# yccyenchicheng/p2pvg

Measured on NVIDIA H100. Metric: frames/sec (train step, device-timed) MovingMNIST 64x64 seq30, higher is better.
Workload: dtype bf16

## Files before the change

### include/p2pvg_b200.h

```cpp
#ifndef P2PVG_B200_H
#define P2PVG_B200_H
#include <stddef.h>
#include <stdint.h>

#ifdef __cplusplus
extern "C" {
#endif
struct p2pvg_conv_fusion;

#define P2PVG_OK 0
#define P2PVG_ERR_BAD_ARG -1
#define P2PVG_ERR_UNSUPPORTED -2
#define P2PVG_ERR_CUDA -3
#define P2PVG_ERR_WORKSPACE -4

#define P2PVG_F32 0
#define P2PVG_BF16 1

#define P2PVG_ACT_NONE 0
#define P2PVG_ACT_LRELU 1
#define P2PVG_ACT_TANH 2
#define P2PVG_ACT_RELU 4
#define P2PVG_ACT_SIGMOID 3

// ... 27 lines not shown
  int act;
} p2pvg_conv_fusion_t;

int p2pvg_im2col3(const void* x, void* col, int dtype, int N, int H, int W, int C, int ld, int sgn, void* stream);
int p2pvg_col2im3(const void* col, void* y, int dtype, int N, int H, int W, int C, int ld, const float* bias, void* stream);
int p2pvg_maxpool2_fwd(const void* x, void* y, int dtype, int N, int H, int W, int C, void* stream);
int p2pvg_maxpool2_bwd(const void* x, const void* dy, void* dx, int dtype, int N, int H, int W, int C, void* stream);
int p2pvg_upsample2_fwd(const void* x, void* y, int dtype, int N, int H, int W, int C, void* stream);
int p2pvg_upsample2_bwd(const void* dy, void* dx, int dtype, int N, int H, int W, int C, void* stream);
int p2pvg_gather_add(void* dst, int dtype, const float* src, const int* grp_src, int G, int64_t n, void* stream);

int p2pvg_conv_thin_in(const void* x, int dtype, const float* w, const float* bias, void* y, int N, int H, int W, int Ci, int Co,
                       void* stream);
int p2pvg_convT_thin_out(const void* x, int dtype, const float* w, const float* bias, const float* addend, const int* grp_src,
                         int imgs_per_group, void* y, int y_dtype, int N, int H, int W, int Ci, int Co, void* stream);

int p2pvg_im2col_k4s2p1(const void* x, void* col, int dtype, int N, int H, int W, int C, void* stream);
int p2pvg_col2im_k4s2p1(const void* col, const void* col2, const int* grp_src, int imgs_per_group, void* y, int dtype, int N,
                        int Hi, int Wi, int C, const float* bias, int accumulate, void* stream);
int p2pvg_permute4(const void* src, int src_dtype, void* dst, int dst_dtype, const int* dims ,
                   const int64_t* src_strides , int accumulate, void* stream);
int p2pvg_nchw_to_nhwc_dual(const float* src, float* dst_f32, void* dst_act, int act_dtype, int64_t N, int hw, int C, void* stream);
int p2pvg_add_indexed(void* dst, const void* src, int dtype, const int* dst_idx, int F, int64_t n, void* stream);
int p2pvg_group_sum(const void* in, void* out, int dtype, const int* grp_src, int G, int F, int64_t n, void* stream);
int p2pvg_transpose_batched(const void* src, int src_dtype, void* dst, int dst_dtype, int A, int P, int Q, void* stream);
int p2pvg_blockdiag(const void* src, int src_dtype, void* dst, int dst_dtype, int R, int C, int g, void* stream);

size_t p2pvg_bn_workspace_bytes(int G, int C);
int p2pvg_bn_fwd_stats(const void* x, int dtype, int G, int64_t R, int C, const float* gamma, const float* beta, float eps,
                       void* ws, size_t ws_bytes, float* mean, float* invstd, float* var_unbiased, float* scale, float* shift,
// ... 96 lines not shown
```

### p2pvg_b200/_lib.py

```python
from __future__ import annotations

import ctypes
import os

import torch

_HERE = os.path.dirname(os.path.abspath(__file__))
LIB_PATH = os.path.join(_HERE, "libp2pvg_b200.so")

F32, BF16 = 0, 1
ACT_NONE, ACT_LRELU, ACT_TANH, ACT_SIGMOID, ACT_RELU = 0, 1, 2, 3, 4

_lib = None


class KernelError(RuntimeError):
    pass


def load_library():
    global _lib
    if _lib is None:
        if not os.path.exists(LIB_PATH):
            raise ImportError(
# ... 150 lines not shown
            fusion = ctypes.byref(ConvFusion(fwd_stat_partial=stat_partial.data_ptr() if stat_partial is not None else None,
                                             addend_dtype=_dt(addend) if addend is not None else F32,
                                             eval_scale=eval_scale.data_ptr() if eval_scale is not None else None,
                                             eval_shift=eval_shift.data_ptr() if eval_shift is not None else None, act=int(act)))
        self._ck(self.lib.p2pvg_conv_gemm(_i(kind), _p(a), _p(b), _i64(ldb), _p(c), _i(_dt(c)), _i64(ldc), _i(N), _i(H), _i(W), _i(Ck),
                                          _i(Cn), _i(Cm), _p(bias), _p(addend), _p(grp_src), _i(imgs_per_group), _i(int(accumulate)),
                                          _p(ws), _sz(ws.numel()), fusion, self._stream()))

    def conv_thin_in(self, x, w, bias, y, N, H, W, Ci, Co):
        self._ck(self.lib.p2pvg_conv_thin_in(_p(x), _i(_dt(x)), _p(w), _p(bias), _p(y), _i(N), _i(H), _i(W), _i(Ci), _i(Co), self._stream()))

    def convT_thin_out(self, x, w, bias, y, N, H, W, Ci, Co, addend=None, grp_src=None, imgs_per_group=0):
        self._ck(self.lib.p2pvg_convT_thin_out(_p(x), _i(_dt(x)), _p(w), _p(bias), _p(addend), _p(grp_src), _i(imgs_per_group), _p(y),
                                               _i(_dt(y)), _i(N), _i(H), _i(W), _i(Ci), _i(Co), self._stream()))

    def im2col(self, x, col, N, H, W, C):
        self._ck(self.lib.p2pvg_im2col_k4s2p1(_p(x), _p(col), _i(_dt(x)), _i(N), _i(H), _i(W), _i(C), self._stream()))

    def col2im(self, col, y, N, Hi, Wi, C, bias=None, col2=None, grp_src=None, imgs_per_group=0, accumulate=False):
        self._ck(self.lib.p2pvg_col2im_k4s2p1(_p(col), _p(col2), _p(grp_src), _i(imgs_per_group), _p(y), _i(_dt(col)), _i(N),
                                              _i(Hi), _i(Wi), _i(C), _p(bias), _i(int(accumulate)), self._stream()))

    def im2col3(self, x, col, N, H, W, C, ld, sgn=1):
        self._ck(self.lib.p2pvg_im2col3(_p(x), _p(col), _i(_dt(x)), _i(N), _i(H), _i(W), _i(C), _i(ld), _i(sgn), self._stream()))

    def col2im3(self, col, y, N, H, W, C, ld, bias=None):
        self._ck(self.lib.p2pvg_col2im3(_p(col), _p(y), _i(_dt(col)), _i(N), _i(H), _i(W), _i(C), _i(ld), _p(bias), self._stream()))

    def maxpool2_fwd(self, x, y, N, H, W, C):
        self._ck(self.lib.p2pvg_maxpool2_fwd(_p(x), _p(y), _i(_dt(x)), _i(N), _i(H), _i(W), _i(C), self._stream()))
# ... 164 lines not shown
```

### p2pvg_b200/csrc/api.cu

```cuda
#include <stdarg.h>
#include <string.h>

#include "../../include/p2pvg_b200.h"
#include <cstdlib>

#include "common.cuh"

static thread_local char g_err[512] = "";

void p2pvg_set_error(const char* fmt, ...) {
  va_list ap;
  va_start(ap, fmt);
  vsnprintf(g_err, sizeof(g_err), fmt, ap);
  va_end(ap);
}

int p2pvg_check_launch(const char* what) {
  cudaError_t e = cudaPeekAtLastError();
  if (e != cudaSuccess) {
    p2pvg_set_error("%s: %s", what, cudaGetErrorString(e));
    (void)cudaGetLastError();
    return P2PVG_ERR_CUDA;
  }
  return P2PVG_OK;
// ... 8 lines not shown
int p2pvg_gemm_tc_available();
int p2pvg_layernorm_fwd_impl(const float*, const float*, const float*, float*, float*, float*, long long, int, float, cudaStream_t);
int p2pvg_layernorm_bwd_impl(const float*, const float*, const float*, const float*, const float*, float*, float*, float*, long long, int,
                             void*, size_t, cudaStream_t);
int p2pvg_mse_plain_impl(const float*, const float*, const int*, const float*, int, long long, float*, float*, int, cudaStream_t);
int p2pvg_conv_thin_in_impl(const void*, int, const float*, const float*, void*, int, int, int, int, int, cudaStream_t);
int p2pvg_convT_thin_out_impl(const void*, int, const float*, const float*, const float*, const int*, int, void*, int, int, int, int, int,
                              int, cudaStream_t);
int p2pvg_conv_gemm_impl(int, const void*, const void*, long long, void*, int, long long, int, int, int, int, int, int, const float*,
                         const float*, const int*, int, int, void*, size_t, void*, int, const float*, const float*, int, cudaStream_t);
int p2pvg_bn_fwd_finalize_tiles_impl(const void*, int, int, int, int, long long, int, const float*, const float*, float, float*, float*, float*,
                                     float*, float*, cudaStream_t);
int p2pvg_bn_bwd_finalize_tiles_impl(const void*, int, int, int, int, int, float*, float*, cudaStream_t);
int p2pvg_bn_bwd_apply_impl(const void*, const void*, const void*, int, const float*, const float*, const float*, int, long long, int, int,
                            void*, const float*, const float*, const float*, const float*, cudaStream_t);
int p2pvg_im2col_k4s2p1_impl(const void*, void*, int, int, int, int, int, cudaStream_t);
int p2pvg_im2col3_impl(const void*, void*, int, int, int, int, int, int, int, cudaStream_t);
int p2pvg_col2im3_impl(const void*, void*, int, int, int, int, int, int, const float*, cudaStream_t);
int p2pvg_maxpool2_fwd_impl(const void*, void*, int, int, int, int, int, cudaStream_t);
int p2pvg_maxpool2_bwd_impl(const void*, const void*, void*, int, int, int, int, int, cudaStream_t);
int p2pvg_upsample2_fwd_impl(const void*, void*, int, int, int, int, int, cudaStream_t);
int p2pvg_upsample2_bwd_impl(const void*, void*, int, int, int, int, int, cudaStream_t);
int p2pvg_gather_add_impl(void*, int, const float*, const int*, int, long long, cudaStream_t);
int p2pvg_col2im_k4s2p1_impl(const void*, const void*, const int*, int, void*, int, int, int, int, int, const float*, int, cudaStream_t);
int p2pvg_permute4_impl(const void*, int, void*, int, const int*, const long long*, int, cudaStream_t);
int p2pvg_nchw_to_nhwc_dual_impl(const float*, float*, void*, int, long long, int, int, cudaStream_t);
int p2pvg_add_indexed_impl(void*, const void*, int, const int*, int, long long, cudaStream_t);
int p2pvg_group_sum_impl(const void*, void*, int, const int*, int, int, long long, cudaStream_t);
int p2pvg_blockdiag_impl(const void*, int, void*, int, int, int, int, cudaStream_t);
int p2pvg_transpose_batched_impl(const void*, int, void*, int, int, int, int, cudaStream_t);
// ... 88 lines not shown
  P2PVG_REQUIRE(add_dt == P2PVG_F32 || add_dt == P2PVG_BF16, P2PVG_ERR_BAD_ARG, "conv_gemm: bad addend dtype %d", add_dt);
  return p2pvg_conv_gemm_impl(kind, a, b, ldb, c, c_dtype, ldc, N, H, W, Ck, Cn, Cm, bias, reinterpret_cast<const float*>(addend), grp_src,
                              imgs_per_group, accumulate, workspace, ws_bytes, fwd_stat, add_dt, fusion ? fusion->eval_scale : nullptr,
                              fusion ? fusion->eval_shift : nullptr, fusion ? fusion->act : 0, ST);
}

int p2pvg_conv_thin_in(const void* x, int dtype, const float* w, const float* bias, void* y, int N, int H, int W, int Ci, int Co,
                       void* stream) {
  return p2pvg_conv_thin_in_impl(x, dtype, w, bias, y, N, H, W, Ci, Co, ST);
}
int p2pvg_convT_thin_out(const void* x, int dtype, const float* w, const float* bias, const float* addend, const int* grp_src,
                         int imgs_per_group, void* y, int y_dtype, int N, int H, int W, int Ci, int Co, void* stream) {
  return p2pvg_convT_thin_out_impl(x, dtype, w, bias, addend, grp_src, imgs_per_group, y, y_dtype, N, H, W, Ci, Co, ST);
}

int p2pvg_im2col_k4s2p1(const void* x, void* col, int dtype, int N, int H, int W, int C, void* stream) {
  return p2pvg_im2col_k4s2p1_impl(x, col, dtype, N, H, W, C, ST);
}
int p2pvg_col2im_k4s2p1(const void* col, const void* col2, const int* grp_src, int imgs_per_group, void* y, int dtype, int N,
                        int Hi, int Wi, int C, const float* bias, int accumulate, void* stream) {
  return p2pvg_col2im_k4s2p1_impl(col, col2, grp_src, imgs_per_group, y, dtype, N, Hi, Wi, C, bias, accumulate, ST);
}
int p2pvg_permute4(const void* src, int src_dtype, void* dst, int dst_dtype, const int* dims, const int64_t* src_strides,
                   int accumulate, void* stream) {
  return p2pvg_permute4_impl(src, src_dtype, dst, dst_dtype, dims, (const long long*)src_strides, accumulate, ST);
}
int p2pvg_nchw_to_nhwc_dual(const float* src, float* dst_f32, void* dst_act, int act_dtype, int64_t N, int hw, int C, void* stream) {
  return p2pvg_nchw_to_nhwc_dual_impl(src, dst_f32, dst_act, act_dtype, (long long)N, hw, C, ST);
}
int p2pvg_add_indexed(void* dst, const void* src, int dtype, const int* dst_idx, int F, int64_t n, void* stream) {
// ... 168 lines not shown
```

### p2pvg_b200/csrc/bn.cu

```cuda
#include "common.cuh"

#define BN_MAXCHUNK 64

namespace {

__device__ __forceinline__ float act_grad(float y, int act) {
  if (act == P2PVG_ACT_LRELU) return y > 0.f ? 1.f : 0.2f;
  if (act == P2PVG_ACT_TANH) return 1.f - y * y;
  return 1.f;
}

template <typename T, int MODE>
__global__ void __launch_bounds__(256, 3) bn_reduce_kernel(const T* __restrict__ x, const T* __restrict__ dy, const T* __restrict__ y,
                                                        const float* __restrict__ mean, const float* __restrict__ invstd, int act,
                                                        long long R, int C, int rows_per_chunk, double2* __restrict__ partial,
                                                        const float* __restrict__ scale, const float* __restrict__ shift) {
  constexpr int V = VecN<T>::N;
  const int CV = C / V;
  const int lanes = 256 / CV;
  const int cv = threadIdx.x % CV, lane = threadIdx.x / CV;
  const int g = blockIdx.y, chunk = blockIdx.x, nchunk = gridDim.x;
  const long long r0 = (long long)chunk * rows_per_chunk;
  long long r1 = r0 + rows_per_chunk;
  if (r1 > R) r1 = R;
// ... 358 lines not shown
                "bn_bwd: y may only be omitted for LeakyReLU with scale/shift supplied");
  const int vec = dtype == P2PVG_BF16 ? 8 : 4;
  if (int e = check_bn_shape(C, vec, "bn_bwd")) return e;
  P2PVG_REQUIRE(ws_bytes >= p2pvg_bn_workspace_bytes_impl(G, C), P2PVG_ERR_WORKSPACE, "bn_bwd: workspace too small");
  if (G == 0) return P2PVG_OK;
  Chunking ch = choose_chunks(R, C, vec);
  dim3 grid(ch.nchunk, G);
  DISPATCH_DTYPE(dtype, T, (bn_reduce_kernel<T, 1><<<grid, 256, 0, st>>>((const T*)x, (const T*)dy, (const T*)y, mean, invstd, act, R, C,
                                                                         ch.rows_per_chunk, (double2*)ws, scale, shift)));
  bn_bwd_finalize_kernel<<<cdiv((long long)G * C, 256), 256, 0, st>>>((const double2*)ws, ch.nchunk, G, C, sum_dz, sum_dzx);
  DISPATCH_DTYPE(dtype, T, (bn_bwd_apply_kernel<T><<<grid, 256, 0, st>>>((const T*)dy, (const T*)x, (const T*)y, mean, invstd, gamma, sum_dz,
                                                                         sum_dzx, R, C, ch.rows_per_chunk, act, (T*)dx, scale, shift)));
  return p2pvg_check_launch("bn_bwd");
}

int p2pvg_bn_param_grad_impl(const float* sum_dz, const float* sum_dzx, int G, int C, float* dgamma, float* dbeta, cudaStream_t st) {
  bn_param_grad_kernel<<<cdiv(C, 128), 128, 0, st>>>(sum_dz, sum_dzx, G, C, dgamma, dbeta);
  return p2pvg_check_launch("bn_param_grad");
}

int p2pvg_bn_ema_impl(float* rmean, float* rvar, const float* mean, const float* var_unbiased, const int* order, int ncalls, int C,
                      float momentum, cudaStream_t st) {
  bn_ema_kernel<<<cdiv(C, 128), 128, 0, st>>>(rmean, rvar, mean, var_unbiased, order, ncalls, C, momentum);
  return p2pvg_check_launch("bn_ema");
}

int p2pvg_bn_eval_coeffs_impl(const float* gamma, const float* beta, const float* rmean, const float* rvar, float eps, int C, float* scale,
                              float* shift, cudaStream_t st) {
  bn_eval_coeffs_kernel<<<cdiv(C, 128), 128, 0, st>>>(gamma, beta, rmean, rvar, eps, C, scale, shift);
  return p2pvg_check_launch("bn_eval_coeffs");
// ... 38 lines not shown
```

### p2pvg_b200/engine.py

```python
from __future__ import annotations

import math
import os
import time
from collections import OrderedDict

import numpy as np
import torch

ACT_NONE, ACT_LRELU, ACT_TANH = 0, 1, 2
BN_MOMENTUM = 0.1


def skip_schedule(seq_len, probs, skip_prob, n_past):
    cp_ix = seq_len - 1
    prev_i, skip_count, out = 0, 0, []
    max_skip = seq_len * skip_prob
    for i in range(1, seq_len):
        if probs[i - 1] <= skip_prob and i >= n_past and skip_count < max_skip and i != 1 and i != cp_ix:
            skip_count += 1
            continue
        out.append((i, (cp_ix - i + 1) / cp_ix, (i - prev_i) / cp_ix))
        prev_i = i
    return out
# ... 112 lines not shown
            self.arena[m] = ParamArena(params[m], self.dev, pool=self.pool)
            self.buffers[m] = {k: v.detach().clone().to(self.dev) for k, v in state[m].items() if not is_param_key(k)}
        self._bufs = {}
        self._buf_gen = 0
        self._plans, self._uploaded = {}, None
        self._packed = {}
        self._graphs = {}
        self.dist = None
        self.tc_lstm = tc_lstm
        import os
        self.thin = hasattr(kernels, "conv_thin_in") and os.environ.get("P2PVG_THIN", "0") == "1"
        r512 = self.R == 512 and tc_lstm and os.environ.get("P2PVG_LSTM_CLUSTER", "1") != "0"
        self.fused_scan = hasattr(kernels, "lstm_scan_fwd") and self.R % 64 == 0 and (self.R <= 256 or r512) and os.environ.get("P2PVG_FUSED_SCAN", "1") != "0"
        self.implicit = (act_dtype == torch.bfloat16) and hasattr(kernels, "conv_gemm") and os.environ.get("P2PVG_IMPLICIT", "1") != "0"
        self.bd = (act_dtype == torch.bfloat16) and hasattr(kernels, "blockdiag") and os.environ.get("P2PVG_BLOCKDIAG", "1") != "0"
        self.addend_dtype = act_dtype if os.environ.get("P2PVG_ADDEND_BF16", "1") != "0" else torch.float32
        self.fuse_last = hasattr(kernels, "convt_c1_loss") and act_dtype == torch.bfloat16 and os.environ.get("P2PVG_FUSE_LAST", "1") != "0"
        self.fuse_stats = self.implicit and os.environ.get("P2PVG_BN_FUSE", "1") != "0"
        self.fuse_stats_min = int(os.environ.get("P2PVG_BN_FUSE_MIN", str(2048 * 128)))
        self.overlap = getattr(kernels, "name", "") == "cuda" and os.environ.get("P2PVG_OVERLAP", "0") == "1"
        self.concurrent = getattr(kernels, "name", "") == "cuda" and act_dtype == torch.bfloat16 and os.environ.get("P2PVG_CONCURRENT", "1") != "0" \
            and os.environ.get("P2PVG_LSTM_CLUSTER", "1") != "0"
        self.streams, self._dirty, self._serial = {}, set(), False
        self.early_loss = getattr(kernels, "name", "") == "cuda" and hasattr(kernels, "publish_scalars") \
            and os.environ.get("P2PVG_EARLY_LOSS", "1") != "0"
        self._pub_seq = 0
        if self.early_loss:
            self._pub_host = torch.zeros(8, dtype=torch.float32).pin_memory()
            self._pub_np = self._pub_host.numpy()
            self._pub_seq_np = self._pub_np.view(np.int32)
# ... 65 lines not shown
            return "upc1.0", "upc1.1"
        if k < self.n - 1:
            return f"upc{k + 2}.main.0", f"upc{k + 2}.main.1"
        return f"upc{self.n + 1}.0", None

    def pack_weights(self, which=("encoder", "decoder")):
        K = self.K
        if "encoder" in which:
            P = self.arena["encoder"].p
            for l in range(self.n + 1):
                w = P[self.enc_names(l)[0] + ".weight"]
                co, ci = w.shape[0], w.shape[1]
                wp = self.buf(f"wp_enc{l}", co * 16 * ci)
                K.transpose_batched(w, wp, co, ci, 16)
                self._packed[f"enc{l}"] = wp
                if self.bd and l == 0 and (16 * ci) % 64 != 0:
                    bd = self.buf("wbd_enc0", 4 * co * 64 * ci)
                    K.blockdiag(wp, bd, co, 16 * ci, 4)
                    b4 = self.fbuf("bias4_enc0", 4 * co)
                    K.permute4(P[self.enc_names(l)[0] + ".bias"], b4, (4, co, 1, 1), (0, 1, 0, 0))
                    self._packed["enc0.bd"], self._packed["enc0.bias4"] = bd, b4
        if "decoder" in which:
            P = self.arena["decoder"].p
            for k in range(-1, self.n):
                cn = self.dec_names(k)[0]
                w = P[cn + ".weight"]
                ci, co = w.shape[0], w.shape[1]
                wp = self.buf(f"wp_dec{k}", ci * 16 * co)
                K.transpose_batched(w, wp, ci, co, 16)
                self._packed[f"dec{k}"] = wp
                if self.bd and k == self.n - 1 and (16 * co) % 64 != 0:
# ... 257 lines not shown
        return a

    def encode(self, x, plan):
        K, T, B, n, nc, W0 = self.K, self.T, self.B, self.n, self.nc, self.W0
        P = self.arena["encoder"].p
        N = T * B
        a = self.frames_nhwc(x)
        self.enc_in = a
        self.enc = []
        H = W0
        for l in range(n):
            cin = nc if l == 0 else self.chans[l - 1]
            cout = self.chans[l]
            Ho = H // 2
            M = N * Ho * Ho
            raw = self.buf(f"enc_raw{l}", M * cout)
            y = self.buf(f"enc_y{l}", M * cout)
            cn, bn = self.enc_names(l)
            imp = self.implicit and cin % 64 == 0 and cout % 64 == 0
            col = None
            thin = self.thin and cin <= 4
            sp = None
            if imp:
                sp = self.stat_buf(f"enc{l}", M, 1, cout, B * Ho * Ho, kred=16 * cin)
                K.conv_gemm(0, a, self._packed[f"enc{l}"], raw, N, Ho, Ho, cin, cout, bias=P[cn + ".bias"],
                            stat_partial=sp["buf"] if sp else None)
            elif thin:
                K.conv_thin_in(a, P[cn + ".weight"], P[cn + ".bias"], raw, N, H, H, cin, cout)
            else:
                col = self.buf(f"enc_col{l}", M * 16 * cin)
                K.im2col(a, col, N, H, H, cin)
                if l == 0 and "enc0.bd" in self._packed:
                    K.gemm(col, self._packed["enc0.bd"], raw, M // 4, 4 * cout, 64 * cin, bias=self._packed["enc0.bias4"])
                else:
                    K.gemm(col, self._packed[f"enc{l}"], raw, M, cout, 16 * cin, bias=P[cn + ".bias"])
            st = self.bn_forward("enc", l, raw, y, T, B * Ho * Ho, cout, P[bn + ".weight"], P[bn + ".bias"], ACT_LRELU, tiles=sp)
            self.enc.append(dict(col=col, raw=raw, y=y, st=st, cin=cin, cout=cout, Hin=H, Hout=Ho, M=M, imp=imp, inp=a, thin=thin))
            a, H = y, Ho
        ctop = self.chans[-1]
        cn, bn = self.enc_names(n)
        raw = self.buf("enc_rawf", N * self.g)
        y = self.buf("enc_yf", N * self.g)
        K.gemm(a, self._packed[f"enc{n}"], raw, N, self.g, 16 * ctop, bias=P[cn + ".bias"])
        st = self.bn_forward("enc", n, raw, y, T, B, self.g, P[bn + ".weight"], P[bn + ".bias"], ACT_TANH)
        self.enc_final = dict(inp=a, raw=raw, y=y, st=st)
        if self.adt == torch.float32:
            self.Hlat = y
        else:
            self.Hlat = self.fbuf("Hlat", N * self.g)
            K.permute4(y, self.Hlat, (N * self.g, 1, 1, 1), (1, 0, 0, 0))
        ncalls = len(plan.enc_order)
        Bf = self.buffers["encoder"]
        for l in range(n + 1):
            st = self.enc[l]["st"] if l < n else self.enc_final["st"]
            bn = self.enc_names(l)[1]
            K.bn_ema(Bf[bn + ".running_mean"], Bf[bn + ".running_var"], st["mean"], st["varu"], self.ix["enc_order"], ncalls,
                     st["C"], BN_MOMENTUM)
            Bf[bn + ".num_batches_tracked"] += ncalls

    def stat_buf(self, tag, rows, phases, C, rows_per_group, kred=1 << 30):
        bn_tile = 256 if C % 256 == 0 else 128 if C > 64 else 64
        if not self.fuse_stats or rows_per_group % 128 != 0 or rows % 128 != 0 or kred * bn_tile < self.fuse_stats_min:
            return None
        buf = self.fbuf(f"bnpart_{tag}", (rows // 128) * phases * C * 2)
        return dict(buf=buf, parts_per_group=(rows_per_group // 128) * phases, ldp=C, fold=1)

    def bn_forward(self, tag, idx, raw, y, G, R, C, gamma, beta, act, tiles=None):
        K = self.K
        names = ("mean", "invstd", "varu", "scale", "shift", "sdz", "sdzx")
        st = {nm: self.fbuf(f"{tag}_bn{idx}_{nm}", G * C) for nm in names}
        st.update(G=G, R=R, C=C, act=act, gamma=gamma)
        if tiles is not None:
            K.bn_fwd_finalize_tiles(tiles["buf"], tiles["parts_per_group"], tiles["ldp"], tiles["fold"], G, R, C, gamma, beta,
                                    st["mean"], st["invstd"], st["varu"], st["scale"], st["shift"])
        else:
            K.bn_fwd_stats(raw, G, R, C, gamma, beta, st["mean"], st["invstd"], st["varu"], st["scale"], st["shift"])
        K.bn_act(raw, y, st["scale"], st["shift"], G, R, C, act)
        return st

    def in_pitch(self, in_dim):
        return (in_dim + 7) // 8 * 8 if self.tc_lstm else in_dim

    def lstm_layers(self, m):
        return len({k.split(".")[1] for k in self.arena[m].p if k.startswith("lstm.")})

    def lstm_forward(self, m, X, steps, in_dim):
# ... 423 lines not shown
        ctop = self.chans[-1]
        gw = self.fbuf(f"gwp_enc{n}", g * 16 * ctop)
        K.gemm(dy, fin["inp"], gw, g, 16 * ctop, N, a_mn=True, b_mn=True, lda=g, ldb=16 * ctop)
        K.transpose_batched(gw, A.g[cn + ".weight"], g, 16, ctop)
        gy = self.buf(f"enc_gy{n - 1}", N * 16 * ctop)
        K.gemm(dy, self._packed[f"enc{n}"], gy, N, 16 * ctop, g, b_mn=True)
        for l in range(n - 1, -1, -1):
            rec = self.enc[l]
            cin, cout, M, Ho = rec["cin"], rec["cout"], rec["M"], rec["Hout"]
            k = n - 1 - l
            dsk = self.dec[k].get("dskip")
            if dsk is not None:
                K.add_indexed(gy, dsk, self.ix["skip_dst"], nskip, B * Ho * Ho * cout)
            cn, bn = self.enc_names(l)
            st = rec["st"]
            self.bn_backward(gy, rec["raw"], rec["y"], st, 0, T * cout, T, B * Ho * Ho, cout, ACT_LRELU)
            K.bn_param_grad(st["sdz"], st["sdzx"], T, cout, A.g[bn + ".weight"], A.g[bn + ".bias"])
            A.g[cn + ".bias"].zero_()
            gw = self.fbuf(f"gwp_enc{l}", cout * 16 * cin)
            if rec["imp"]:
                with self.fork(self.LANE_WGRAD, heavy=True):
                    K.conv_gemm(1, gy, rec["inp"], gw, N, Ho, Ho, 0, cin, Cm=cout)
                    K.transpose_batched(gw, A.g[cn + ".weight"], cout, 16, cin)
            else:
                col = rec["col"]
                if col is None:
                    col = self.buf(f"enc_col{l}", M * 16 * cin)
                    K.im2col(rec["inp"], col, N, rec["Hin"], rec["Hin"], cin)
                K.gemm(gy, col, gw, cout, 16 * cin, M, a_mn=True, b_mn=True, lda=cout, ldb=16 * cin)
            if not rec["imp"]:
                K.transpose_batched(gw, A.g[cn + ".weight"], cout, 16, cin)
# ... 86 lines not shown
```

Measured before the change: 199,600.

## Fuse first encoder conv with BatchNorm and LeakyReLU via recompute

Adds a dedicated tensor-core kernel for the first (1-channel) encoder conv. In the forward pass it computes the conv twice: once to gather BatchNorm statistics, and once to apply the normalisation and LeakyReLU and write only the activation. In the backward pass it recomputes the conv again to produce the BN input gradient in two passes, so the raw pre-BN tensor, the im2col buffer and the blockdiag GEMM are never materialised. This trades extra conv arithmetic on a very thin input for less memory traffic and fewer launches.

Measured after the change: 209,300, median of 6. +4.9%, better.

```diff
diff --git a/include/p2pvg_b200.h b/include/p2pvg_b200.h
--- a/include/p2pvg_b200.h
+++ b/include/p2pvg_b200.h
@@ -65,6 +65,14 @@
                        void* stream);
 int p2pvg_convT_thin_out(const void* x, int dtype, const float* w, const float* bias, const float* addend, const int* grp_src,
                          int imgs_per_group, void* y, int y_dtype, int N, int H, int W, int Ci, int Co, void* stream);
+
+int p2pvg_enc_first_schedule(int N, int H, int W, int cin, int G, int max_ctas, int* out);
+int p2pvg_enc_first_fwd(const void* x, const void* w, const float* bias, int N, int H, int W, int cin, int G, const float* gamma,
+                        const float* beta, float eps, void* bn_ws, size_t bn_ws_bytes, float* mean, float* invstd, float* var_unbiased,
+                        float* scale, float* shift, void* y, int max_ctas, void* stream);
+int p2pvg_enc_first_bwd(const void* x, const void* w, const float* bias, void* gy, int N, int H, int W, int cin, int G,
+                        const float* mean, const float* invstd, const float* gamma, const float* scale, const float* shift, void* bn_ws,
+                        size_t bn_ws_bytes, float* sum_dz, float* sum_dzx, int max_ctas, void* stream);
 
 int p2pvg_im2col_k4s2p1(const void* x, void* col, int dtype, int N, int H, int W, int C, void* stream);
 int p2pvg_col2im_k4s2p1(const void* col, const void* col2, const int* grp_src, int imgs_per_group, void* y, int dtype, int N,
diff --git a/p2pvg_b200/_lib.py b/p2pvg_b200/_lib.py
--- a/p2pvg_b200/_lib.py
+++ b/p2pvg_b200/_lib.py
@@ -188,6 +188,24 @@
         self._ck(self.lib.p2pvg_convT_thin_out(_p(x), _i(_dt(x)), _p(w), _p(bias), _p(addend), _p(grp_src), _i(imgs_per_group), _p(y),
                                                _i(_dt(y)), _i(N), _i(H), _i(W), _i(Ci), _i(Co), self._stream()))
 
+    def enc_first_schedule(self, N, H, W, cin, G, max_ctas=0):
+        out = (_i * 3)()
+        self._ck(self.lib.p2pvg_enc_first_schedule(_i(N), _i(H), _i(W), _i(cin), _i(G), _i(max_ctas), out))
+        self.launches -= 1
+        return tuple(out)
+
+    def enc_first_fwd(self, x, w, bias, N, H, W, cin, G, gamma, beta, mean, invstd, var_unb, scale, shift, y, eps=1e-5, max_ctas=0):
+        ws = self.bn_workspace(G, 64)
+        self._ck(self.lib.p2pvg_enc_first_fwd(_p(x), _p(w), _p(bias), _i(N), _i(H), _i(W), _i(cin), _i(G), _p(gamma), _p(beta), _f(eps),
+                                              _p(ws), _sz(ws.numel()), _p(mean), _p(invstd), _p(var_unb), _p(scale), _p(shift), _p(y),
+                                              _i(max_ctas), self._stream()))
+
+    def enc_first_bwd(self, x, w, bias, gy, N, H, W, cin, G, mean, invstd, gamma, scale, shift, sum_dz, sum_dzx, max_ctas=0):
+        bws = self.bn_workspace(G, 64)
+        self._ck(self.lib.p2pvg_enc_first_bwd(_p(x), _p(w), _p(bias), _p(gy), _i(N), _i(H), _i(W), _i(cin), _i(G), _p(mean), _p(invstd),
+                                              _p(gamma), _p(scale), _p(shift), _p(bws), _sz(bws.numel()), _p(sum_dz), _p(sum_dzx),
+                                              _i(max_ctas), self._stream()))
+
     def im2col(self, x, col, N, H, W, C):
         self._ck(self.lib.p2pvg_im2col_k4s2p1(_p(x), _p(col), _i(_dt(x)), _i(N), _i(H), _i(W), _i(C), self._stream()))
 
diff --git a/p2pvg_b200/csrc/api.cu b/p2pvg_b200/csrc/api.cu
--- a/p2pvg_b200/csrc/api.cu
+++ b/p2pvg_b200/csrc/api.cu
@@ -46,6 +46,11 @@
 int p2pvg_bn_bwd_finalize_tiles_impl(const void*, int, int, int, int, int, float*, float*, cudaStream_t);
 int p2pvg_bn_bwd_apply_impl(const void*, const void*, const void*, int, const float*, const float*, const float*, int, long long, int, int,
                             void*, const float*, const float*, const float*, const float*, cudaStream_t);
+int p2pvg_enc_first_schedule_impl(int, int, int, int, int, int, int*);
+int p2pvg_enc_first_fwd_impl(const void*, const void*, const float*, int, int, int, int, int, const float*, const float*, float, void*, size_t,
+                             float*, float*, float*, float*, float*, void*, int, cudaStream_t);
+int p2pvg_enc_first_bwd_impl(const void*, const void*, const float*, void*, int, int, int, int, int, const float*, const float*,
+                             const float*, const float*, const float*, void*, size_t, float*, float*, int, cudaStream_t);
 int p2pvg_im2col_k4s2p1_impl(const void*, void*, int, int, int, int, int, cudaStream_t);
 int p2pvg_im2col3_impl(const void*, void*, int, int, int, int, int, int, int, cudaStream_t);
 int p2pvg_col2im3_impl(const void*, void*, int, int, int, int, int, int, const float*, cudaStream_t);
@@ -164,6 +169,22 @@
   return p2pvg_convT_thin_out_impl(x, dtype, w, bias, addend, grp_src, imgs_per_group, y, y_dtype, N, H, W, Ci, Co, ST);
 }
 
+int p2pvg_enc_first_schedule(int N, int H, int W, int cin, int G, int max_ctas, int* out) {
+  return p2pvg_enc_first_schedule_impl(N, H, W, cin, G, max_ctas, out);
+}
+int p2pvg_enc_first_fwd(const void* x, const void* w, const float* bias, int N, int H, int W, int cin, int G, const float* gamma,
+                        const float* beta, float eps, void* bn_ws, size_t bn_ws_bytes, float* mean, float* invstd, float* var_unbiased,
+                        float* scale, float* shift, void* y, int max_ctas, void* stream) {
+  return p2pvg_enc_first_fwd_impl(x, w, bias, N, H, W, cin, G, gamma, beta, eps, bn_ws, bn_ws_bytes, mean, invstd, var_unbiased, scale, shift,
+                                  y, max_ctas, ST);
+}
+int p2pvg_enc_first_bwd(const void* x, const void* w, const float* bias, void* gy, int N, int H, int W, int cin, int G,
+                        const float* mean, const float* invstd, const float* gamma, const float* scale, const float* shift, void* bn_ws,
+                        size_t bn_ws_bytes, float* sum_dz, float* sum_dzx, int max_ctas, void* stream) {
+  return p2pvg_enc_first_bwd_impl(x, w, bias, gy, N, H, W, cin, G, mean, invstd, gamma, scale, shift, bn_ws, bn_ws_bytes, sum_dz, sum_dzx,
+                                  max_ctas, ST);
+}
+
 int p2pvg_im2col_k4s2p1(const void* x, void* col, int dtype, int N, int H, int W, int C, void* stream) {
   return p2pvg_im2col_k4s2p1_impl(x, col, dtype, N, H, W, C, ST);
 }
diff --git a/p2pvg_b200/csrc/bn.cu b/p2pvg_b200/csrc/bn.cu
--- a/p2pvg_b200/csrc/bn.cu
+++ b/p2pvg_b200/csrc/bn.cu
@@ -396,6 +396,18 @@
   return p2pvg_check_launch("bn_bwd");
 }
 
+int p2pvg_bn_fwd_finalize_chunks_impl(const void* partial, int nchunk, int G, int C, long long R, const float* gamma, const float* beta,
+                                      float eps, float* mean, float* invstd, float* var_unbiased, float* scale, float* shift, cudaStream_t st) {
+  bn_fwd_finalize_kernel<<<cdiv((long long)G * C, 256), 256, 0, st>>>((const double2*)partial, nchunk, G, C, R, gamma, beta, eps, mean,
+                                                                      invstd, var_unbiased, scale, shift);
+  return p2pvg_check_launch("bn_fwd_finalize");
+}
+
+int p2pvg_bn_bwd_finalize_chunks_impl(const void* partial, int nchunk, int G, int C, float* sum_dz, float* sum_dzx, cudaStream_t st) {
+  bn_bwd_finalize_kernel<<<cdiv((long long)G * C, 256), 256, 0, st>>>((const double2*)partial, nchunk, G, C, sum_dz, sum_dzx);
+  return p2pvg_check_launch("bn_bwd_finalize");
+}
+
 int p2pvg_bn_param_grad_impl(const float* sum_dz, const float* sum_dzx, int G, int C, float* dgamma, float* dbeta, cudaStream_t st) {
   bn_param_grad_kernel<<<cdiv(C, 128), 128, 0, st>>>(sum_dz, sum_dzx, G, C, dgamma, dbeta);
   return p2pvg_check_launch("bn_param_grad");
diff --git a/p2pvg_b200/csrc/enc_first.cu b/p2pvg_b200/csrc/enc_first.cu
--- /dev/null
+++ b/p2pvg_b200/csrc/enc_first.cu
@@ -0,0 +1,435 @@
+#include "common.cuh"
+
+namespace {
+
+constexpr int EF_CO = 64;
+constexpr int EF_WARPS = 8;
+constexpr int EF_THREADS = EF_WARPS * 32;
+constexpr int EF_MAXCHUNK = 64;
+constexpr int EF_LANES = 32;
+
+struct EFArgs {
+  const bf16* x;
+  const bf16* w;
+  const float* bias;
+  bf16* gy;
+  bf16* y;
+  int H, W, tiles_per_row, tiles_per_img, tiles_per_group;
+  int nchunk, tiles_per_chunk, chunks, units;
+  const float *mean, *invstd, *gamma, *scale, *shift, *sum_dz, *sum_dzx;
+  float invR;
+  double2* partial;
+};
+
+__device__ __forceinline__ void mma_bf16(float* c, const uint32_t* a, uint32_t b0, uint32_t b1) {
+  asm("mma.sync.aligned.m16n8k16.row.col.f32.bf16.bf16.f32 {%0,%1,%2,%3}, {%4,%5,%6,%7}, {%8,%9}, {%0,%1,%2,%3};\n"
+      : "+f"(c[0]), "+f"(c[1]), "+f"(c[2]), "+f"(c[3])
+      : "r"(a[0]), "r"(a[1]), "r"(a[2]), "r"(a[3]), "r"(b0), "r"(b1));
+}
+
+__device__ __forceinline__ uint32_t pack_bf16(float lo, float hi) {
+  __nv_bfloat162 p = __floats2bfloat162_rn(lo, hi);
+  return *reinterpret_cast<uint32_t*>(&p);
+}
+__device__ __forceinline__ float bf16_lo(uint32_t v) { return __uint_as_float(v << 16); }
+__device__ __forceinline__ float bf16_hi(uint32_t v) { return __uint_as_float(v & 0xffff0000u); }
+__device__ __forceinline__ float round_bf16(float v) { return __bfloat162float(__float2bfloat16_rn(v)); }
+
+__device__ __forceinline__ uint32_t tile_addr(uint32_t base, int r, int c) { return base + r * 128 + ((c ^ (r & 7)) << 4); }
+
+__device__ __forceinline__ uint32_t frag_row_addr(uint32_t base, int lane, int i) {
+  const int mm = lane >> 3;
+  return tile_addr(base, 8 * (mm >> 1) + (lane & 7), 2 * i + (mm & 1));
+}
+__device__ __forceinline__ void ldsm_x4_t(uint32_t* r, uint32_t addr) {
+  asm volatile("ldmatrix.sync.aligned.m8n8.x4.trans.shared.b16 {%0,%1,%2,%3}, [%4];\n"
+               : "=r"(r[0]), "=r"(r[1]), "=r"(r[2]), "=r"(r[3]) : "r"(addr) : "memory");
+}
+__device__ __forceinline__ void stsm_x4_t(uint32_t addr, const uint32_t* r) {
+  asm volatile("stmatrix.sync.aligned.m8n8.x4.trans.shared.b16 [%0], {%1,%2,%3,%4};\n"
+               :: "r"(addr), "r"(r[0]), "r"(r[1]), "r"(r[2]), "r"(r[3]) : "memory");
+}
+__device__ __forceinline__ void lds128(uint4& v, uint32_t addr) {
+  asm volatile("ld.shared.v4.u32 {%0,%1,%2,%3}, [%4];\n" : "=r"(v.x), "=r"(v.y), "=r"(v.z), "=r"(v.w) : "r"(addr) : "memory");
+}
+__device__ __forceinline__ void sts128(uint32_t addr, const uint4& v) {
+  asm volatile("st.shared.v4.u32 [%0], {%1,%2,%3,%4};\n" :: "r"(addr), "r"(v.x), "r"(v.y), "r"(v.z), "r"(v.w) : "memory");
+}
+
+template <int CI>
+__device__ __forceinline__ uint32_t tap(const unsigned short* __restrict__ xi, int H, int W, int oy, int ox, int k) {
+  const int t = k / CI, ci = k - t * CI;
+  const int iy = 2 * oy - 1 + (t >> 2), ix = 2 * ox - 1 + (t & 3);
+  return (iy >= 0 && iy < H && ix >= 0 && ix < W) ? (uint32_t)__ldg(xi + (iy * W + ix) * CI + ci) : 0u;
+}
+
+template <int CI, int PASS>
+__global__ void __launch_bounds__(EF_THREADS, CI == 1 && PASS != 2 ? 2 : 1) enc_first_kernel(const EFArgs p) {
+  constexpr int KS = CI;
+  constexpr int K = 16 * CI;
+  constexpr bool WREG = CI == 1;
+  constexpr bool STATS = PASS == 0 || PASS == 2;
+  __shared__ uint4 wfrag[WREG ? 1 : 4 * KS * 32];
+  __shared__ __align__(128) unsigned char tiles[EF_WARPS][16 * 128];
+  __shared__ float sbias[EF_CO];
+  __shared__ float4 prm[EF_WARPS / 2][2][EF_CO];
+  __shared__ double2 carry[STATS ? EF_WARPS / 2 : 1][EF_CO];
+
+  const int lane = threadIdx.x & 31, warp = threadIdx.x >> 5;
+  const int g = lane >> 2, t = lane & 3;
+  const int slot = warp >> 1, parity = warp & 1;
+  const uint32_t sbase = (uint32_t)__cvta_generic_to_shared(&tiles[warp][0]);
+
+  uint32_t wa[4][WREG ? KS : 1][4];
+  const uint32_t* w32 = reinterpret_cast<const uint32_t*>(p.w);
+#pragma unroll
+  for (int i = 0; i < 4; i++)
+#pragma unroll
+    for (int s = 0; s < KS; s++) {
+      uint32_t f[4];
+#pragma unroll
+      for (int q = 0; q < 4; q++) f[q] = __ldg(w32 + ((16 * i + g + 8 * (q & 1)) * K + 16 * s + 2 * t + 8 * (q >> 1)) / 2);
+      if (WREG) {
+#pragma unroll
+        for (int q = 0; q < 4; q++) wa[i][WREG ? s : 0][q] = f[q];
+      } else if (warp == 0) {
+        wfrag[WREG ? 0 : (i * KS + s) * 32 + lane] = make_uint4(f[0], f[1], f[2], f[3]);
+      }
+    }
+  if (threadIdx.x < EF_CO) sbias[threadIdx.x] = p.bias[threadIdx.x];
+  __syncthreads();
+
+  const unsigned short* xs = reinterpret_cast<const unsigned short*>(p.x);
+  const int img_elems = p.H * p.W * CI;
+
+  for (int u = blockIdx.x; u < p.units; u += gridDim.x) {
+    const int q = u * (EF_WARPS / 2) + slot;
+    const bool live = q < p.chunks;
+    const int grp = live ? q / p.nchunk : 0, chunk = live ? q - grp * p.nchunk : 0;
+    const int t0 = grp * p.tiles_per_group + chunk * p.tiles_per_chunk;
+    int t1 = t0 + p.tiles_per_chunk;
+    if (t1 > (grp + 1) * p.tiles_per_group) t1 = (grp + 1) * p.tiles_per_group;
+    if (!live) t1 = t0;
+    if (PASS != 0) {
+      __syncthreads();
+      if (parity == 0 && live) {
+        for (int c = lane; c < EF_CO; c += 32) {
+          const int gc = grp * EF_CO + c;
+          const float mu = p.mean[gc], is = p.invstd[gc];
+          prm[slot][0][c] = make_float4(p.scale[gc], p.shift[gc], mu, is);
+          if (PASS == 3) prm[slot][1][c] = make_float4(p.gamma[c] * is, p.sum_dz[gc] * p.invR, p.sum_dzx[gc] * p.invR, 0.f);
+        }
+      }
+      __syncthreads();
+    }
+    float s0[4][2][2][2], s1[4][2][2][2];
+#pragma unroll
+    for (int i = 0; i < 4; i++)
+#pragma unroll
+      for (int h = 0; h < 2; h++)
+#pragma unroll
+        for (int j = 0; j < 2; j++)
+#pragma unroll
+          for (int e = 0; e < 2; e++) s0[i][h][j][e] = s1[i][h][j][e] = 0.f;
+
+    int tile = t0 + parity;
+    uint4 gbuf[4];
+    auto load_gy = [&](int tl) {
+      const uint4* src = reinterpret_cast<const uint4*>(p.gy + (size_t)tl * 16 * EF_CO);
+#pragma unroll
+      for (int r = 0; r < 4; r++) gbuf[r] = __ldcs(src + r * 32 + lane);
+    };
+    if (PASS >= 2 && tile < t1) load_gy(tile);
+    for (; tile < t1; tile += 2) {
+      const int n = tile / p.tiles_per_img;
+      const int rem = tile - n * p.tiles_per_img;
+      const int oy = rem / p.tiles_per_row, ox0 = (rem - oy * p.tiles_per_row) * 16;
+      const unsigned short* xi = xs + (size_t)n * img_elems;
+
+      if (PASS >= 2) {
+#pragma unroll
+        for (int r = 0; r < 4; r++) {
+          const int idx = r * 32 + lane;
+          sts128(tile_addr(sbase, idx >> 3, idx & 7), gbuf[r]);
+        }
+        __syncwarp();
+        if (tile + 2 < t1) load_gy(tile + 2);
+      }
+      uint32_t bf[2][KS][2];
+#pragma unroll
+      for (int j = 0; j < 2; j++) {
+        const int ox = ox0 + 8 * j + g;
+#pragma unroll
+        for (int s = 0; s < KS; s++) {
+          const int k = 16 * s + 2 * t;
+          bf[j][s][0] = tap<CI>(xi, p.H, p.W, oy, ox, k) | (tap<CI>(xi, p.H, p.W, oy, ox, k + 1) << 16);
+          bf[j][s][1] = tap<CI>(xi, p.H, p.W, oy, ox, k + 8) | (tap<CI>(xi, p.H, p.W, oy, ox, k + 9) << 16);
+        }
+      }
+
+#pragma unroll
+      for (int i = 0; i < 4; i++) {
+        float c[2][4];
+#pragma unroll
+        for (int j = 0; j < 2; j++) {
+#pragma unroll
+          for (int r = 0; r < 4; r++) c[j][r] = 0.f;
+#pragma unroll
+          for (int s = 0; s < KS; s++) {
+            if (WREG) {
+              mma_bf16(c[j], wa[i][WREG ? s : 0], bf[j][s][0], bf[j][s][1]);
+            } else {
+              const uint4 f = wfrag[WREG ? 0 : (i * KS + s) * 32 + lane];
+              const uint32_t fa[4] = {f.x, f.y, f.z, f.w};
+              mma_bf16(c[j], fa, bf[j][s][0], bf[j][s][1]);
+            }
+          }
+        }
+        uint32_t gv[4];
+        if (PASS >= 2) ldsm_x4_t(gv, frag_row_addr(sbase, lane, i));
+        float bs[2];
+        float4 pa[2], pb[2];
+#pragma unroll
+        for (int h = 0; h < 2; h++) {
+          bs[h] = sbias[16 * i + g + 8 * h];
+          if (PASS != 0) pa[h] = prm[slot][0][16 * i + g + 8 * h];
+          if (PASS == 3) pb[h] = prm[slot][1][16 * i + g + 8 * h];
+        }
+        uint32_t out[4];
+#pragma unroll
+        for (int j = 0; j < 2; j++) {
+          float o[4];
+#pragma unroll
+          for (int r = 0; r < 4; r++) {
+            const int h = r >> 1, e = r & 1;
+            const float x = round_bf16(c[j][r] + bs[h]);
+            if (PASS == 0) {
+              s0[i][h][j][e] += x;
+              s1[i][h][j][e] = fmaf(x, x, s1[i][h][j][e]);
+            } else if (PASS == 1) {
+              float z = fmaf(x, pa[h].x, pa[h].y);
+              z = z > 0.f ? z : 0.2f * z;
+              o[r] = z;
+            } else {
+              const uint32_t gw = gv[2 * j + h];
+              const float dv = e ? bf16_hi(gw) : bf16_lo(gw);
+              const float xhat = (x - pa[h].z) * pa[h].w;
+              const float ya = fmaf(x, pa[h].x, pa[h].y);
+              const float dz = dv * (ya > 0.f ? 1.f : 0.2f);
+              if (PASS == 2) {
+                s0[i][h][j][e] += dz;
+                s1[i][h][j][e] = fmaf(dz, xhat, s1[i][h][j][e]);
+              } else {
+                o[r] = pb[h].x * (dz - pb[h].y - xhat * pb[h].z);
+              }
+            }
+          }
+          if (PASS == 1 || PASS == 3) {
+            out[2 * j] = pack_bf16(o[0], o[1]);
+            out[2 * j + 1] = pack_bf16(o[2], o[3]);
+          }
+        }
+        if (PASS == 1 || PASS == 3) stsm_x4_t(frag_row_addr(sbase, lane, i), out);
+      }
+
+      if (PASS == 1 || PASS == 3) {
+        __syncwarp();
+        uint4* dst = reinterpret_cast<uint4*>((PASS == 1 ? p.y : p.gy) + (size_t)tile * 16 * EF_CO);
+#pragma unroll
+        for (int r = 0; r < 4; r++) {
+          const int idx = r * 32 + lane;
+          uint4 v;
+          lds128(v, tile_addr(sbase, idx >> 3, idx & 7));
+          dst[r * 32 + lane] = v;
+        }
+      }
+      __syncwarp();
+    }
+
+    if (STATS && parity == 0) {
+#pragma unroll
+      for (int i = 0; i < 4; i++)
+#pragma unroll
+        for (int h = 0; h < 2; h++) {
+          double a = 0.0, b = 0.0;
+#pragma unroll
+          for (int px = 0; px < 16; px++) {
+            const int j = px >> 3, e = px & 1, src = (g << 2) | ((px >> 1) & 3);
+            a += (double)__shfl_sync(0xffffffffu, s0[i][h][j][e], src);
+            b += (double)__shfl_sync(0xffffffffu, s1[i][h][j][e], src);
+          }
+          if (t == 0) carry[STATS ? slot : 0][16 * i + g + 8 * h] = make_double2(a, b);
+        }
+    }
+    if (STATS) __syncthreads();
+    if (STATS && parity == 1 && live) {
+#pragma unroll
+      for (int i = 0; i < 4; i++)
+#pragma unroll
+        for (int h = 0; h < 2; h++) {
+          const int c = 16 * i + g + 8 * h;
+          const double2 cr = carry[STATS ? slot : 0][c];
+          double a = cr.x, b = cr.y;
+#pragma unroll
+          for (int px = 0; px < 16; px++) {
+            const int j = px >> 3, e = px & 1, src = (g << 2) | ((px >> 1) & 3);
+            a += (double)__shfl_sync(0xffffffffu, s0[i][h][j][e], src);
+            b += (double)__shfl_sync(0xffffffffu, s1[i][h][j][e], src);
+          }
+          if (t == 0) p.partial[((long long)grp * p.nchunk + chunk) * EF_CO + c] = make_double2(a, b);
+        }
+    }
+  }
+}
+
+struct EFSchedule {
+  int tiles_per_row, tiles_per_img, tiles_per_group, nchunk, tiles_per_chunk, chunks, units, rows_per_chunk;
+  long long tiles, R;
+};
+
+EFSchedule schedule(int N, int H, int W, int G) {
+  EFSchedule s;
+  const int Ho = H / 2, Wo = W / 2;
+  s.tiles_per_row = Wo / 16;
+  s.tiles_per_img = Ho * s.tiles_per_row;
+  s.tiles = (long long)N * s.tiles_per_img;
+  s.tiles_per_group = (int)(s.tiles / G);
+  s.R = (long long)s.tiles_per_group * 16;
+  long long want = (s.R + (long long)EF_LANES * 16 - 1) / ((long long)EF_LANES * 16);
+  s.nchunk = (int)(want < 1 ? 1 : (want > EF_MAXCHUNK ? EF_MAXCHUNK : want));
+  s.rows_per_chunk = (int)((s.R + s.nchunk - 1) / s.nchunk);
+  s.nchunk = (int)((s.R + s.rows_per_chunk - 1) / s.rows_per_chunk);
+  s.tiles_per_chunk = s.rows_per_chunk / 16;
+  s.chunks = G * s.nchunk;
+  s.units = (s.chunks + EF_WARPS / 2 - 1) / (EF_WARPS / 2);
+  return s;
+}
+
+int device_sms() {
+  static int sms = 0;
+  if (sms == 0) {
+    int dev = 0, v = 0;
+    if (cudaGetDevice(&dev) == cudaSuccess && cudaDeviceGetAttribute(&v, cudaDevAttrMultiProcessorCount, dev) == cudaSuccess && v > 0)
+      sms = v;
+    else
+      sms = 132;
+  }
+  return sms;
+}
+
+template <int CI, int PASS>
+int grid_of(int units, int max_ctas) {
+  static int per_sm = 0;
+  if (per_sm == 0) {
+    int v = 0;
+    if (cudaOccupancyMaxActiveBlocksPerMultiprocessor(&v, enc_first_kernel<CI, PASS>, EF_THREADS, 0) != cudaSuccess || v < 1) v = 1;
+    per_sm = v;
+  }
+  int cap = per_sm * device_sms();
+  if (max_ctas > 0 && max_ctas < cap) cap = max_ctas;
+  const int rounds = (units + cap - 1) / cap;
+  return (units + rounds - 1) / rounds;
+}
+
+template <int PASS>
+int launch(int cin, const EFArgs& a, int max_ctas, cudaStream_t st) {
+  if (cin == 1) enc_first_kernel<1, PASS><<<grid_of<1, PASS>(a.units, max_ctas), EF_THREADS, 0, st>>>(a);
+  else enc_first_kernel<3, PASS><<<grid_of<3, PASS>(a.units, max_ctas), EF_THREADS, 0, st>>>(a);
+  return p2pvg_check_launch("enc_first");
+}
+
+int check_shape(int N, int H, int W, int cin, int G, const char* what) {
+  P2PVG_REQUIRE(cin == 1 || cin == 3, P2PVG_ERR_UNSUPPORTED, "%s: %d input channels (1 or 3 supported)", what, cin);
+  P2PVG_REQUIRE(N > 0 && G > 0 && N % G == 0, P2PVG_ERR_BAD_ARG, "%s: %d frames are not %d equal groups", what, N, G);
+  P2PVG_REQUIRE(H % 2 == 0 && W % 32 == 0 && H >= 2, P2PVG_ERR_UNSUPPORTED, "%s: %dx%d frames (need an even height and W/2 a multiple of 16)",
+                what, H, W);
+  P2PVG_REQUIRE((long long)N * H * W * 64 / 4 < (1LL << 31), P2PVG_ERR_UNSUPPORTED, "%s: more than 2^31 output elements", what);
+  const EFSchedule s = schedule(N, H, W, G);
+  P2PVG_REQUIRE(s.rows_per_chunk % 16 == 0, P2PVG_ERR_UNSUPPORTED, "%s: BatchNorm chunks of %d rows are not whole 16-pixel tiles", what,
+                s.rows_per_chunk);
+  return P2PVG_OK;
+}
+
+int check(const void* x, const void* w, const float* bias, int N, int H, int W, int cin, int G, const char* what) {
+  P2PVG_REQUIRE(x && w && bias, P2PVG_ERR_BAD_ARG, "%s: null operand", what);
+  P2PVG_REQUIRE((reinterpret_cast<uintptr_t>(w) & 3) == 0, P2PVG_ERR_BAD_ARG, "%s: weight not 4-byte aligned", what);
+  return check_shape(N, H, W, cin, G, what);
+}
+
+EFArgs make_args(const void* x, const void* w, const float* bias, int H, int W, const EFSchedule& s) {
+  EFArgs a{};
+  a.x = (const bf16*)x;
+  a.w = (const bf16*)w;
+  a.bias = bias;
+  a.H = H;
+  a.W = W;
+  a.tiles_per_row = s.tiles_per_row;
+  a.tiles_per_img = s.tiles_per_img;
+  a.tiles_per_group = s.tiles_per_group;
+  a.nchunk = s.nchunk;
+  a.tiles_per_chunk = s.tiles_per_chunk;
+  a.chunks = s.chunks;
+  a.units = s.units;
+  a.invR = 1.f / (float)s.R;
+  return a;
+}
+
+}
+
+int p2pvg_bn_fwd_finalize_chunks_impl(const void* partial, int nchunk, int G, int C, long long R, const float* gamma, const float* beta,
+                                      float eps, float* mean, float* invstd, float* var_unbiased, float* scale, float* shift, cudaStream_t st);
+int p2pvg_bn_bwd_finalize_chunks_impl(const void* partial, int nchunk, int G, int C, float* sum_dz, float* sum_dzx, cudaStream_t st);
+
+int p2pvg_enc_first_schedule_impl(int N, int H, int W, int cin, int G, int max_ctas, int* out) {
+  P2PVG_REQUIRE(out, P2PVG_ERR_BAD_ARG, "enc_first_schedule: null output");
+  if (int e = check_shape(N, H, W, cin, G, "enc_first_schedule")) return e;
+  const EFSchedule s = schedule(N, H, W, G);
+  out[0] = (int)s.tiles;
+  out[1] = s.units;
+  out[2] = cin == 1 ? grid_of<1, 0>(s.units, max_ctas) : grid_of<3, 0>(s.units, max_ctas);
+  return P2PVG_OK;
+}
+
+int p2pvg_enc_first_fwd_impl(const void* x, const void* w, const float* bias, int N, int H, int W, int cin, int G, const float* gamma,
+                             const float* beta, float eps, void* ws, size_t ws_bytes, float* mean, float* invstd, float* var_unbiased,
+                             float* scale, float* shift, void* y, int max_ctas, cudaStream_t st) {
+  if (int e = check(x, w, bias, N, H, W, cin, G, "enc_first_fwd")) return e;
+  P2PVG_REQUIRE(y && (reinterpret_cast<uintptr_t>(y) & 15) == 0, P2PVG_ERR_BAD_ARG, "enc_first_fwd: output not 16-byte aligned");
+  const EFSchedule s = schedule(N, H, W, G);
+  P2PVG_REQUIRE(ws && ws_bytes >= (size_t)G * s.nchunk * EF_CO * sizeof(double2), P2PVG_ERR_WORKSPACE, "enc_first_fwd: workspace too small");
+  EFArgs a = make_args(x, w, bias, H, W, s);
+  a.partial = (double2*)ws;
+  a.mean = mean;
+  a.invstd = invstd;
+  a.scale = scale;
+  a.shift = shift;
+  a.y = (bf16*)y;
+  if (int e = launch<0>(cin, a, max_ctas, st)) return e;
+  if (int e = p2pvg_bn_fwd_finalize_chunks_impl(ws, s.nchunk, G, EF_CO, s.R, gamma, beta, eps, mean, invstd, var_unbiased, scale, shift, st))
+    return e;
+  return launch<1>(cin, a, max_ctas, st);
+}
+
+int p2pvg_enc_first_bwd_impl(const void* x, const void* w, const float* bias, void* gy, int N, int H, int W, int cin, int G,
+                             const float* mean, const float* invstd, const float* gamma, const float* scale, const float* shift, void* bn_ws,
+                             size_t bn_ws_bytes, float* sum_dz, float* sum_dzx, int max_ctas, cudaStream_t st) {
+  if (int e = check(x, w, bias, N, H, W, cin, G, "enc_first_bwd")) return e;
+  P2PVG_REQUIRE(gy && (reinterpret_cast<uintptr_t>(gy) & 15) == 0, P2PVG_ERR_BAD_ARG, "enc_first_bwd: gradient not 16-byte aligned");
+  P2PVG_REQUIRE(sum_dz && sum_dzx, P2PVG_ERR_BAD_ARG, "enc_first_bwd: null output");
+  const EFSchedule s = schedule(N, H, W, G);
+  P2PVG_REQUIRE(bn_ws && bn_ws_bytes >= (size_t)G * s.nchunk * EF_CO * sizeof(double2), P2PVG_ERR_WORKSPACE,
+                "enc_first_bwd: BatchNorm workspace too small");
+  EFArgs a = make_args(x, w, bias, H, W, s);
+  a.gy = (bf16*)gy;
+  a.partial = (double2*)bn_ws;
+  a.mean = mean;
+  a.invstd = invstd;
+  a.gamma = gamma;
+  a.scale = scale;
+  a.shift = shift;
+  a.sum_dz = sum_dz;
+  a.sum_dzx = sum_dzx;
+  if (int e = launch<2>(cin, a, max_ctas, st)) return e;
+  if (int e = p2pvg_bn_bwd_finalize_chunks_impl(bn_ws, s.nchunk, G, EF_CO, sum_dz, sum_dzx, st)) return e;
+  return launch<3>(cin, a, max_ctas, st);
+}
diff --git a/p2pvg_b200/engine.py b/p2pvg_b200/engine.py
--- a/p2pvg_b200/engine.py
+++ b/p2pvg_b200/engine.py
@@ -150,6 +150,8 @@
         self.fused_scan = hasattr(kernels, "lstm_scan_fwd") and self.R % 64 == 0 and (self.R <= 256 or r512) and os.environ.get("P2PVG_FUSED_SCAN", "1") != "0"
         self.implicit = (act_dtype == torch.bfloat16) and hasattr(kernels, "conv_gemm") and os.environ.get("P2PVG_IMPLICIT", "1") != "0"
         self.bd = (act_dtype == torch.bfloat16) and hasattr(kernels, "blockdiag") and os.environ.get("P2PVG_BLOCKDIAG", "1") != "0"
+        self.enc_first = (act_dtype == torch.bfloat16) and hasattr(kernels, "enc_first_fwd") and self.backbone == "dcgan" \
+            and self.nc == 1
         self.addend_dtype = act_dtype if os.environ.get("P2PVG_ADDEND_BF16", "1") != "0" else torch.float32
         self.fuse_last = hasattr(kernels, "convt_c1_loss") and act_dtype == torch.bfloat16 and os.environ.get("P2PVG_FUSE_LAST", "1") != "0"
         self.fuse_stats = self.implicit and os.environ.get("P2PVG_BN_FUSE", "1") != "0"
@@ -245,7 +247,7 @@
                 wp = self.buf(f"wp_enc{l}", co * 16 * ci)
                 K.transpose_batched(w, wp, co, ci, 16)
                 self._packed[f"enc{l}"] = wp
-                if self.bd and l == 0 and (16 * ci) % 64 != 0:
+                if self.bd and l == 0 and not self.enc_first and (16 * ci) % 64 != 0:
                     bd = self.buf("wbd_enc0", 4 * co * 64 * ci)
                     K.blockdiag(wp, bd, co, 16 * ci, 4)
                     b4 = self.fbuf("bias4_enc0", 4 * co)
@@ -533,28 +535,32 @@
             cout = self.chans[l]
             Ho = H // 2
             M = N * Ho * Ho
-            raw = self.buf(f"enc_raw{l}", M * cout)
             y = self.buf(f"enc_y{l}", M * cout)
             cn, bn = self.enc_names(l)
             imp = self.implicit and cin % 64 == 0 and cout % 64 == 0
-            col = None
-            thin = self.thin and cin <= 4
-            sp = None
-            if imp:
-                sp = self.stat_buf(f"enc{l}", M, 1, cout, B * Ho * Ho, kred=16 * cin)
-                K.conv_gemm(0, a, self._packed[f"enc{l}"], raw, N, Ho, Ho, cin, cout, bias=P[cn + ".bias"],
-                            stat_partial=sp["buf"] if sp else None)
-            elif thin:
-                K.conv_thin_in(a, P[cn + ".weight"], P[cn + ".bias"], raw, N, H, H, cin, cout)
+            first = l == 0 and self.enc_first
+            rec = dict(col=None, raw=None, y=y, cin=cin, cout=cout, Hin=H, Hout=Ho, M=M, imp=imp, inp=a, first=first)
+            if first:
+                st = self.bn_stats("enc", l, T, B * Ho * Ho, cout, P[bn + ".weight"], ACT_LRELU)
+                K.enc_first_fwd(a, self._packed["enc0"], P[cn + ".bias"], N, H, H, cin, T, P[bn + ".weight"], P[bn + ".bias"],
+                                st["mean"], st["invstd"], st["varu"], st["scale"], st["shift"], y)
             else:
-                col = self.buf(f"enc_col{l}", M * 16 * cin)
-                K.im2col(a, col, N, H, H, cin)
-                if l == 0 and "enc0.bd" in self._packed:
-                    K.gemm(col, self._packed["enc0.bd"], raw, M // 4, 4 * cout, 64 * cin, bias=self._packed["enc0.bias4"])
+                raw = rec["raw"] = self.buf(f"enc_raw{l}", M * cout)
+                sp = None
+                if imp:
+                    sp = self.stat_buf(f"enc{l}", M, 1, cout, B * Ho * Ho, kred=16 * cin)
+                    K.conv_gemm(0, a, self._packed[f"enc{l}"], raw, N, Ho, Ho, cin, cout, bias=P[cn + ".bias"],
+                                stat_partial=sp["buf"] if sp else None)
                 else:
-                    K.gemm(col, self._packed[f"enc{l}"], raw, M, cout, 16 * cin, bias=P[cn + ".bias"])
-            st = self.bn_forward("enc", l, raw, y, T, B * Ho * Ho, cout, P[bn + ".weight"], P[bn + ".bias"], ACT_LRELU, tiles=sp)
-            self.enc.append(dict(col=col, raw=raw, y=y, st=st, cin=cin, cout=cout, Hin=H, Hout=Ho, M=M, imp=imp, inp=a, thin=thin))
+                    col = rec["col"] = self.buf(f"enc_col{l}", M * 16 * cin)
+                    K.im2col(a, col, N, H, H, cin)
+                    if l == 0 and "enc0.bd" in self._packed:
+                        K.gemm(col, self._packed["enc0.bd"], raw, M // 4, 4 * cout, 64 * cin, bias=self._packed["enc0.bias4"])
+                    else:
+                        K.gemm(col, self._packed[f"enc{l}"], raw, M, cout, 16 * cin, bias=P[cn + ".bias"])
+                st = self.bn_forward("enc", l, raw, y, T, B * Ho * Ho, cout, P[bn + ".weight"], P[bn + ".bias"], ACT_LRELU, tiles=sp)
+            rec["st"] = st
+            self.enc.append(rec)
             a, H = y, Ho
         ctop = self.chans[-1]
         cn, bn = self.enc_names(n)
@@ -584,11 +590,15 @@
         buf = self.fbuf(f"bnpart_{tag}", (rows // 128) * phases * C * 2)
         return dict(buf=buf, parts_per_group=(rows_per_group // 128) * phases, ldp=C, fold=1)
 
-    def bn_forward(self, tag, idx, raw, y, G, R, C, gamma, beta, act, tiles=None):
-        K = self.K
+    def bn_stats(self, tag, idx, G, R, C, gamma, act):
         names = ("mean", "invstd", "varu", "scale", "shift", "sdz", "sdzx")
         st = {nm: self.fbuf(f"{tag}_bn{idx}_{nm}", G * C) for nm in names}
         st.update(G=G, R=R, C=C, act=act, gamma=gamma)
+        return st
+
+    def bn_forward(self, tag, idx, raw, y, G, R, C, gamma, beta, act, tiles=None):
+        K = self.K
+        st = self.bn_stats(tag, idx, G, R, C, gamma, act)
         if tiles is not None:
             K.bn_fwd_finalize_tiles(tiles["buf"], tiles["parts_per_group"], tiles["ldp"], tiles["fold"], G, R, C, gamma, beta,
                                     st["mean"], st["invstd"], st["varu"], st["scale"], st["shift"])
@@ -1042,7 +1052,11 @@
                 K.add_indexed(gy, dsk, self.ix["skip_dst"], nskip, B * Ho * Ho * cout)
             cn, bn = self.enc_names(l)
             st = rec["st"]
-            self.bn_backward(gy, rec["raw"], rec["y"], st, 0, T * cout, T, B * Ho * Ho, cout, ACT_LRELU)
+            if rec["first"]:
+                K.enc_first_bwd(rec["inp"], self._packed["enc0"], A.p[cn + ".bias"], gy, N, rec["Hin"], rec["Hin"], cin, T,
+                                st["mean"], st["invstd"], st["gamma"], st["scale"], st["shift"], st["sdz"], st["sdzx"])
+            else:
+                self.bn_backward(gy, rec["raw"], rec["y"], st, 0, T * cout, T, B * Ho * Ho, cout, ACT_LRELU)
             K.bn_param_grad(st["sdz"], st["sdzx"], T, cout, A.g[bn + ".weight"], A.g[bn + ".bias"])
             A.g[cn + ".bias"].zero_()
             gw = self.fbuf(f"gwp_enc{l}", cout * 16 * cin)
```
